# chairclr/PathTracing

Hardware: AMD Instinct MI355X
Metric: Mrays/s (higher is better)
Workload: dtype f32

## Files before the change

pathtracing_amd/csrc/kernels.hip:

```cpp
#include "ptrt_internal.h"
#include "pt_device.h"
#include <algorithm>
#include <cstdlib>


using namespace ptd;

namespace ptrt {

PT_DEV uint32_t lane_prefix(uint64_t m) { return __builtin_amdgcn_mbcnt_hi((uint32_t)(m >> 32), __builtin_amdgcn_mbcnt_lo((uint32_t)m, 0u)); }
PT_DEV uint32_t lane_id() { return lane_prefix(~0ull); }

typedef const float4 __attribute__((address_space(4))) *uniform_f4;
PT_DEV uniform_f4 as_uniform(const float4 *p) { return (uniform_f4)(uintptr_t)p; }
PT_DEV float4 uniform_load(uniform_f4 p, uint32_t i) { return make_float4(p[i].x, p[i].y, p[i].z, p[i].w); }
PT_DEV uint32_t spheres_test(const float4 *spheres, uint32_t n_spheres, uint32_t first_id, V3 o, V3 d, Hit &h)
{
    const uniform_f4 sp = as_uniform(spheres);
    for (uint32_t j = 0; j < n_spheres; j += 4u) {
        const float4 s0 = uniform_load(sp, j), s1 = uniform_load(sp, j + 1u), s2 = uniform_load(sp, j + 2u), s3 = uniform_load(sp, j + 3u);
        sphere_test(s0, first_id + j, o, d, h);
        if (j + 1u < n_spheres) sphere_test(s1, first_id + j + 1u, o, d, h);
        if (j + 2u < n_spheres) sphere_test(s2, first_id + j + 2u, o, d, h);
        if (j + 3u < n_spheres) sphere_test(s3, first_id + j + 3u, o, d, h);
// ... 300 lines not shown
    const bool in_range = j < ps.shard_cap && slot < ps.n_slots;
    const uint32_t first = first_sample(slot, fp);
    const bool valid = in_range && first < fp.spp && slot_pixel(slot, fp, x, y);
    if (in_range && !fp.accumulate) ps.acc[slot] = make_float4(0.f, 0.f, 0.f, 0.f);
    if (valid && full == 1u) {
        PathRegs r;
        path_init(sc, fp, slot, r);
        path_store(ps, slot, r);
    }
    if (full == 2u) wave_push(&ps.counters[cnt_ext_index(0, shard)], ps.q_ext[0] + (size_t)shard * ps.shard_cap, valid, slot);
    else if (j < ps.shard_cap) ps.q_ext[0][(size_t)shard * ps.shard_cap + j] = valid ? slot : kInvalidSlot;
    const uint32_t n_alive = (uint32_t)__syncthreads_count(valid);
    if (threadIdx.x == 0) {
        if (n_alive) atomicAdd(&ps.counters[cnt_alive_index(0, shard)], n_alive);
        if (bx == 0 && full != 2u) ps.counters[cnt_ext_index(0, shard)] = ps.shard_cap;
    }
}


template <int MODE>
PT_DEV bool shade_one(const DeviceScene &sc, const PathState &ps, const FrameParams &fp, uint32_t slot, PathRegs &r, float t, uint32_t ref,
                      uint32_t b, uint32_t &defer)
{
    V3 &o = r.o, &d = r.d, &T = r.T;
    uint32_t &key = r.key, &sample = r.sample;
    uint32_t depth = r.depth + 1u;
    float4 A = at(ps.acc, slot);
    bool touched = false, term = false, alive = false;
    auto add = [&](V3 L) {
        touched = true;
        A.x = fma_(T.x, L.x, A.x); A.y = fma_(T.y, L.y, A.y); A.z = fma_(T.z, L.z, A.z);
    };

    if (ref == PT_MISS) {
        add(v3(sc.sky[0], sc.sky[1], sc.sky[2]));
        term = true;
    } else {
        const V3 P = madd(t, d, o);
        V3 ng;
        uint32_t mat;
        if (ref < sc.n_tris) {
            const float4 ts = sc.tris[(size_t)ref * 4 + 3];
            ng = xyz(ts);
            mat = __float_as_uint(ts.w);
        } else {
            const uint32_t j = ref - sc.n_tris;
            const float4 s = sc.spheres[j];
            const uint2 mi = sc.sph_mat[j];
            const float ir = __uint_as_float(mi.y);
            ng = v3((P.x - s.x) * ir, (P.y - s.y) * ir, (P.z - s.z) * ir);
            mat = mi.x;
        }
        const bool front = dot(ng, d) < 0.0f;
        const V3 n = front ? ng : neg(ng);
        float4 m0 = sc.mats[(size_t)mat * 3], m1 = sc.mats[(size_t)mat * 3 + 1];
        const float4 m2 = sc.mats[(size_t)mat * 3 + 2];
        asm volatile("" : "+v"(m0.x), "+v"(m1.x));
        const V3 alb = v3(m0.y, m0.z, m0.w), emi = xyz(m1);
        const uint32_t kind = __float_as_uint(m0.x);
        if (MODE == SHADE_QUEUE && kind != (uint32_t)PT_LAMBERT) { defer = 1u + kind; return false; }
        if (emi.x != 0.0f || emi.y != 0.0f || emi.z != 0.0f) add(emi);
        if (depth >= fp.max_depth) term = true;
        else {
            const uint32_t bb = depth - 1u;
            const uint32_t bk = MODE == SHADE_QUEUE ? (uint32_t)B_LAMBERT : MODE == SHADE_BUCKETS ? b : 1u + kind;
            BsdfSample bs;
            if (bk == B_LAMBERT) bs = sample_lambert(alb, n, u01(key, 4u + 4u * bb), u01(key, 5u + 4u * bb));
            else if (bk == B_METAL) bs = sample_metal(alb, m1.w, d, n, u01(key, 4u + 4u * bb), u01(key, 5u + 4u * bb));
            else bs = sample_dielectric(alb, m2.x, d, n, front, u01(key, 6u + 4u * bb));
            const V3 wi = bs.wi, W = bs.W;
            const float side = bs.side;
            if (!bs.ok) term = true;
            else {
                T = v3(T.x * W.x, T.y * W.y, T.z * W.z);
                if (!(fmax_(T.x, fmax_(T.y, T.z)) > 0.0f)) term = true;
                else if (depth >= fp.rr_start) {
                    const float qrr = fmin_(fmax_(T.x, fmax_(T.y, T.z)), 0.95f);
                    if (!(u01(key, 7u + 4u * bb) < qrr)) term = true;
                    else { const float iq = 1.0f / qrr; T = v3(T.x * iq, T.y * iq, T.z * iq); }
                }
                if (!term) { o = madd(side * fp.ray_eps, n, P); d = wi; }
            }
        }
    }

    if (term) {
        touched = true;
        A.w += 1.0f;
        sample += fp.streams;
        if (sample < fp.spp) {
            uint32_t x = 0, y = 0;
            slot_pixel(slot, fp, x, y);
            key = path_key(fp.seed_hashed, y * fp.width + x, fp.sample_offset + sample);
            camera_ray_of(sc.cam, x, y, key, o, d);
            T = v3(1.f, 1.f, 1.f);
            depth = 0;
            alive = true;
        }
    } else alive = true;
    if (touched) at(ps.acc, slot) = A;
    r.depth = depth;
    return alive;
}

PT_DEV unsigned long long *traced_counter(const PathState &ps, uint32_t c, uint32_t shard)
{
    return reinterpret_cast<unsigned long long *>(ps.counters + cnt_traced_index(c, shard));
}
PT_DEV void fold_traced(const PathState &ps, uint32_t shard, uint32_t it, uint32_t n, uint32_t n_alive)
{
    *traced_counter(ps, (it + 2u) % 3u, shard) = 0ull;
    const unsigned long long traced = *traced_counter(ps, it % 3u, shard);
    *reinterpret_cast<unsigned long long *>(ps.counters + cnt_rays_index(shard)) += traced;
    if (ps.host_ring && it) ps.host_ring[((it - 1u) % ps.ring_slots) * kShards + shard] = make_uint4(n, n_alive, (uint32_t)traced, (uint32_t)(traced >> 32));
}

PT_DEV bool want_compact(const PathState &ps, uint32_t len, uint32_t n_alive, uint32_t prev_alive, bool sticky, bool forced)
{
    const uint32_t deaths = prev_alive > n_alive ? prev_alive - n_alive : 0u;
    const uint32_t predicted = n_alive > deaths ? n_alive - deaths : 0u;
    return forced || (sticky && len < ps.shard_cap) || (float)predicted < ps.compact_below * (float)len;
}

PT_DEV void queue_next(const PathState &ps, uint32_t shard, uint32_t cnext, uint32_t *q_next, uint32_t gid, uint32_t total, bool alive,
                       uint32_t slot, bool compact)
{
    if (compact) wave_push(&ps.counters[cnt_ext_index(cnext, shard)], q_next, alive, slot);
    else {
        if (gid < total) at(q_next, gid) = alive ? slot : kInvalidSlot;
        if (gid == 0) ps.counters[cnt_ext_index(cnext, shard)] = total;
    }
    const uint64_t m = __ballot(alive);
    if (m && lane_id() == 0u) atomicAdd(&ps.counters[cnt_alive_index(cnext, shard)], (uint32_t)__popcll(m));
}

#ifndef PT_EXT_WAVES
#define PT_EXT_WAVES(L, FUSE) (((L) == PT_BVH_WIDTH_4Q || (L) == PT_BVH_WIDTH_2) && (FUSE) != SHADE_INLINE ? 8 : 7)
#endif
struct StackCtx { int32_t *lds; uint32_t stride, tid, col; };
PT_DEV void push_slow(const StackCtx &k, uint32_t &sp, int32_t v)
{
    if (sp < kStackLds) k.lds[sp * k.stride + k.tid] = v;
    else {
        const PathState &ps = cold().ps;
        const uint32_t e = sp - kStackLds;
        if (e < ps.stack_ovf_entries) ps.stack_ovf[(size_t)e * ((size_t)kShards * ps.shard_cap) + k.col] = v;
        else { atomicOr(&ps.counters[kCntError], 1u); return; }
    }
    ++sp;
}
PT_DEV int32_t pop_slow(const StackCtx &k, uint32_t &sp)
{
    if (sp == 0) return PT_BVH_EMPTY;
    --sp;
    if (sp < kStackLds) return k.lds[sp * k.stride + k.tid];
    const PathState &ps = cold().ps;
    return ps.stack_ovf[(size_t)(sp - kStackLds) * ((size_t)kShards * ps.shard_cap) + k.col];
}
PT_DEV int32_t pop_lds(const StackCtx &k, uint32_t &sp)
{
    if (sp == 0) return PT_BVH_EMPTY;
    --sp;
    return k.lds[sp * k.stride + k.tid];
}
PT_DEV int32_t pop_after_leaf(const StackCtx &k, uint32_t &sp)
{
    const bool deep = __any((int)(sp > kStackLds)) != 0;
    return deep ? pop_slow(k, sp) : pop_lds(k, sp);
}

template <int L>
PT_DEV void node_visit_rows(const float4 *__restrict__ base, float4 r0, float4 r1, float4 r2, float4 r3, const StackCtx &k, const RaySetup &rs,
                            float t_best, int32_t &cur, uint32_t &sp);
template <int L>
PT_DEV void node_step(const float4 *__restrict__ nodes, const StackCtx &k, const RaySetup &rs, float t_best, int32_t &cur, uint32_t &sp)
{
    const float4 *base = nodes + (size_t)cur * node_rows<L>();
    node_visit_rows<L>(base, base[0], base[1], base[2], base[3], k, rs, t_best, cur, sp);
}
template <int L>
PT_DEV void node_visit_rows(const float4 *__restrict__ base, float4 r0, float4 r1, float4 r2, float4 r3, const StackCtx &k, const RaySetup &rs,
                            float t_best, int32_t &cur, uint32_t &sp)
{
    constexpr int N = fanout<L>();
    const bool deep = __any((int)(sp + (uint32_t)(N - 1) > kStackLds)) != 0;
    if constexpr (L == PT_BVH_WIDTH_8O) {
        uint32_t hits;
        int32_t ref[N];
        visit_node_oct8(base, r0, r1, r2, r3, rs, t_best, hits, ref);
        int32_t prev = PT_BVH_EMPTY;
        if (!deep) {
#pragma unroll
            for (int p = N - 1; p >= 0; --p) {
                const bool h = (hits >> p) & 1u;
                k.lds[sp * k.stride + k.tid] = prev;
                sp += (h && prev != PT_BVH_EMPTY) ? 1u : 0u;
                prev = h ? ref[p] : prev;
            }
            cur = prev != PT_BVH_EMPTY ? prev : pop_lds(k, sp);
        } else {
#pragma unroll
            for (int p = N - 1; p >= 0; --p)
                if ((hits >> p) & 1u) { if (prev != PT_BVH_EMPTY) push_slow(k, sp, prev); prev = ref[p]; }
            cur = prev != PT_BVH_EMPTY ? prev : pop_slow(k, sp);
        }
        return;
    }
    uint32_t key[N];
    int32_t ref[N];
    visit_node<L>(base, r0, r1, r2, r3, rs, t_best, key, ref);
    if (!deep) {
#pragma unroll
        for (int i = N - 1; i >= 1; --i) {
            k.lds[sp * k.stride + k.tid] = ref[i];
            sp += key[i] != 0xFFFFFFFFu ? 1u : 0u;
        }
        cur = key[0] != 0xFFFFFFFFu ? ref[0] : pop_lds(k, sp);
    } else {
#pragma unroll
        for (int i = N - 1; i >= 1; --i)
            if (key[i] != 0xFFFFFFFFu) push_slow(k, sp, ref[i]);
        cur = (key[0] != 0xFFFFFFFFu) ? ref[0] : pop_slow(k, sp);
    }
}

PT_DEV uint32_t leaf_step(const float4 *__restrict__ tris, const StackCtx &k, V3 o, V3 d, Hit &h, int32_t &cur, uint32_t &sp)
{
    const uint32_t enc = (uint32_t)~cur;
    uint32_t first = enc >> 3, more = enc & 7u, n = 0;
    for (;;) {
        const float4 *base = tris + (size_t)first * 4;
        const float4 r0 = base[0], r1 = base[1], r2 = base[2];
        tri_test(r0, r1, r2, first, o, d, h);
        ++n;
        if (more == 0u) break;
        ++first; --more;
    }
    cur = pop_after_leaf(k, sp);
    return n;
}

constexpr uint32_t kFinishVertices = 256;

struct ExtHead {
    uint32_t shard, bx, parity, cnext, n, n_alive;
    bool do_compact, idle;
};
template <int FUSE>
PT_DEV ExtHead extend_head(const ExtArgs &a, const PathState &ps, uint32_t per_block, uint32_t tid, bool predicted, bool carry_len)
{
    ExtHead e;
    const uint32_t it = a.it, ccur = it % 3u, czero = (it + 2u) % 3u;
    e.parity = it & 1u; e.cnext = (it + 1u) % 3u;
    uint32_t nbx;
    block_pos(a.ps, e.shard, e.bx, nbx);
    e.n = ps.counters[cnt_ext_index(ccur, e.shard)]; e.n_alive = ps.counters[cnt_alive_index(ccur, e.shard)];
    e.do_compact = FUSE != SHADE_NONE &&
                   (predicted ? want_compact(ps, e.n, e.n_alive, ps.counters[cnt_prev_alive_index(ccur, e.shard)], ps.repack_sticky != 0u, a.compact != 0u)
                              : want_compact(ps, e.n, e.n_alive, 0u, false, a.compact != 0u));
    if (e.bx * per_block + tid == 0u) {
        ps.counters[cnt_prev_alive_index(e.cnext, e.shard)] = e.n_alive;
        ps.counters[cnt_ext_index(czero, e.shard)] = 0u;
        ps.counters[cnt_alive_index(czero, e.shard)] = 0u;
        fold_traced(ps, e.shard, it, e.n, e.n_alive);
        if (FUSE == SHADE_NONE) *traced_counter(ps, e.cnext, e.shard) = e.n_alive;
        else if (carry_len && !e.do_compact) ps.counters[cnt_ext_index(e.cnext, e.shard)] = e.n;
        if (e.do_compact && e.n_alive) atomicAdd(&ps.counters[kCntCompactions], 1u);
    }
    e.idle = e.bx * per_block >= e.n || e.n_alive == 0u;
    return e;
}

PT_DEV void stash_park(uint32_t *stash, uint32_t stride, uint32_t tid, const PathRegs &r)
{
    stash[0 * stride + tid] = __float_as_uint(r.T.x); stash[1 * stride + tid] = __float_as_uint(r.T.y);
    stash[2 * stride + tid] = __float_as_uint(r.T.z); stash[3 * stride + tid] = r.key;
    stash[4 * stride + tid] = (r.sample << 8) | r.depth;
    asm volatile("" ::: "memory");
}
PT_DEV void stash_restore(const uint32_t *stash, uint32_t stride, uint32_t tid, PathRegs &r)
{
    r.T = v3(__uint_as_float(stash[0 * stride + tid]), __uint_as_float(stash[1 * stride + tid]), __uint_as_float(stash[2 * stride + tid]));
    r.key = stash[3 * stride + tid];
    const uint32_t sdv = stash[4 * stride + tid];
    r.sample = sdv >> 8; r.depth = sdv & 255u;
}

struct VisitCounts {
    unsigned long long nodes = 0, tris = 0, sph = 0;
    unsigned long long wave_iters = 0, wave_iters_late = 0, idle_leaf = 0, idle_done = 0;
};
PT_DEV void flush_visit_counters(const PathState &ps, const VisitCounts &v)
{
    auto add = [&](uint32_t i, unsigned long long x) { atomicAdd(reinterpret_cast<unsigned long long *>(ps.counters + i), x); };
    if (v.wave_iters) add(kCntWaveNodeIters, v.wave_iters);
    if (v.wave_iters_late) add(kCntWaveNodeIters + 2, v.wave_iters_late);
    if (v.idle_leaf) add(kCntIdleLeaf, v.idle_leaf);
    if (v.idle_done) add(kCntIdleDone, v.idle_done);
    add(kCntNodes, v.nodes);
    add(kCntTris, v.tris);
    add(kCntSph, v.sph);
}

template <int L, bool COUNT, int FUSE>
__global__ void __launch_bounds__(kExtBlock) __attribute__((amdgpu_waves_per_eu(PT_EXT_WAVES(L, FUSE), PT_EXT_WAVES(L, FUSE)))) k_extend(ExtArgs a)
{
    const float4 *__restrict__ nodes = a.sc.nodes, *__restrict__ tris = a.sc.tris, *__restrict__ spheres = a.sc.spheres;
    const uint32_t n_spheres = a.sc.n_spheres, n_tris = a.sc.n_tris, n_nodes = a.sc.n_nodes;
    const uint32_t it = a.it;
    __shared__ int32_t s_stack[kStackLds * kExtBlock];
    __shared__ uint32_t s_stash[(FUSE != SHADE_NONE ? 5 : 1) * kExtBlock];
    const uint32_t tid = threadIdx.x;
    ExtHead hd;
    uint32_t gid, qbase, slot = kInvalidSlot, n_bounces;
    {
        const PathState &ps = cold().ps;
        hd = extend_head<FUSE>(a, ps, kExtBlock, tid, true, false);
        gid = hd.bx * kExtBlock + tid;
        if (hd.idle) return;
        qbase = hd.shard * ps.shard_cap;
        if (gid < hd.n) slot = at(ps.q_ext[hd.parity], qbase + gid);
        const bool sparse = hd.do_compact && (float)hd.n_alive < ps.sparse_below * (float)hd.n;
        n_bounces = FUSE == SHADE_NONE ? 1u : (hd.n_alive <= ps.finish_below ? kFinishVertices : sparse ? 1u : a.bounces);
    }
    const uint32_t shard = hd.shard, parity = hd.parity, n = hd.n;
    const bool active = slot != kInvalidSlot;
    const StackCtx stk{ s_stack, kExtBlock, tid, qbase + gid };

    VisitCounts vc;
    __shared__ int32_t s_state[COUNT ? 64 : 1];
    PathRegs r;
    r.o = v3(0.f, 0.f, 0.f); r.d = v3(0.f, 0.f, 1.f); r.T = v3(0.f, 0.f, 0.f); r.key = r.sample = r.depth = 0u;
    if (active) {
        const PathState &ps = cold().ps;
        if (FUSE == SHADE_NONE) { r.o = xyz(at(ps.ray_o, slot)); r.d = xyz(at(ps.ray_d, slot)); }
        else if (it == 0u) {
            path_init(cold().sc, cold().fp, slot, r);
            if (!cold().fp.accumulate) at(ps.acc, slot) = make_float4(0.f, 0.f, 0.f, 0.f);
        }
        else path_load(ps, slot, r);
    }
    bool alive = active;
    uint32_t wave_rays = 0;
    for (uint32_t bounce = 0; bounce < n_bounces; ++bounce) {
    const uint64_t alive_mask = __ballot(alive);
    if (alive_mask == 0) break;
    wave_rays += (uint32_t)__popcll(alive_mask);
    if (COUNT && kExtBlock == 64u) { s_state[tid] = alive ? 0 : 1; __syncthreads(); }
    if (alive) {
        const V3 o = r.o, d = r.d;
        Hit h{ __builtin_inff(), PT_MISS, PT_MISS };
        if (FUSE != SHADE_NONE) stash_park(s_stash, kExtBlock, tid, r);

        { const uint32_t ns = spheres_test(spheres, n_spheres, n_tris, o, d, h); if (COUNT) vc.sph += ns; }

        const RaySetup rs = ray_setup(o, d);
        int32_t cur = n_nodes ? 0 : PT_BVH_EMPTY;
        uint32_t sp = 0, steps = 0;
        if (n_nodes) {
            ++steps;
            if (COUNT) { vc.nodes++; if (lane_id() == (uint32_t)(__ffsll((long long)__ballot(1)) - 1)) vc.wave_iters++; }
            const uniform_f4 root = as_uniform(nodes);
            node_visit_rows<L>(nodes, uniform_load(root, 0), uniform_load(root, 1), uniform_load(root, 2), uniform_load(root, 3), stk, rs, h.t, cur, sp);
            if (COUNT) s_state[tid & 63u] = cur;
        }

        bool late_cycle = false;
        for (;;) {
            while ((uint32_t)cur < (uint32_t)PT_BVH_EMPTY) {
                if (++steps > (1u << 22)) { atomicOr(&cold().ps.counters[kCntError], 2u); cur = PT_BVH_EMPTY; break; }
                if (COUNT) {
                    vc.nodes++;
                    if (lane_id() == (uint32_t)(__ffsll((long long)__ballot(1)) - 1)) {
                        vc.wave_iters++; if (late_cycle) vc.wave_iters_late++;
                        uint32_t n_leaf = 0, n_done = 0;
                        for (uint32_t l = 0; l < 64u; ++l) { const int32_t c2 = s_state[l]; n_leaf += c2 < 0 ? 1u : 0u; n_done += c2 == PT_BVH_EMPTY ? 1u : 0u; }
                        vc.idle_leaf += n_leaf; vc.idle_done += n_done;
                    }
                }
                node_step<L>(nodes, stk, rs, h.t, cur, sp);
                if (COUNT) s_state[tid & 63u] = cur;
            }
            if (cur == PT_BVH_EMPTY) break;
            if (COUNT) late_cycle = true;
            const uint32_t nt = leaf_step(tris, stk, o, d, h, cur, sp);
            if (COUNT) { vc.tris += nt; s_state[tid & 63u] = cur; }
        }

        if (FUSE == SHADE_NONE) at(cold().ps.hit, slot) = make_float2(h.t, __uint_as_float(h.ref));
        else {
            stash_restore(s_stash, kExtBlock, tid, r);
            uint32_t defer = 0u;
            const ExtArgs &c = cold();
            alive = shade_one<FUSE>(c.sc, c.ps, c.fp, slot, r, h.t, h.ref, B_LAMBERT, defer);
        }
    }
    }
    const PathState &ps = cold().ps;
    if (COUNT && active) flush_visit_counters(ps, vc);
    if (FUSE != SHADE_NONE) {
        if (alive) path_store(ps, slot, r);
        queue_next(ps, shard, hd.cnext, &at(ps.q_ext[parity ^ 1u], qbase), gid, n, alive, slot, hd.do_compact);
        if (wave_rays && lane_id() == 0u) atomicAdd(traced_counter(ps, hd.cnext, shard), (unsigned long long)wave_rays);
    }
}


#ifndef PT_REFILL_IDLE
#define PT_REFILL_IDLE 16
#endif
constexpr uint32_t kRefillIdle = PT_REFILL_IDLE;

#ifndef PT_PACKED_WAVES
#define PT_PACKED_WAVES(FUSE) ((FUSE) == SHADE_INLINE ? 6 : 7)
#endif
template <int L, bool COUNT, int FUSE>
__global__ void __launch_bounds__(64) __attribute__((amdgpu_waves_per_eu(PT_PACKED_WAVES(FUSE), PT_PACKED_WAVES(FUSE))))
k_extend_packed(ExtArgs a)
{
    const float4 *__restrict__ nodes = a.sc.nodes, *__restrict__ tris = a.sc.tris, *__restrict__ spheres = a.sc.spheres;
    const uint32_t n_spheres = a.sc.n_spheres, n_tris = a.sc.n_tris, n_nodes = a.sc.n_nodes;
    const uint32_t it = a.it, chunk = a.chunk, bounces = a.bounces;
    __shared__ int32_t s_stack[kStackLds * 64];
    __shared__ uint32_t s_stash[(FUSE != SHADE_NONE ? 5 : 1) * 64];
    const uint32_t lane = threadIdx.x;
    const ExtHead hd = extend_head<FUSE>(a, cold().ps, chunk, lane, false, true);
    if (hd.idle) return;
    const uint32_t shard = hd.shard, n_alive = hd.n_alive;
    const bool do_compact = hd.do_compact;
    uint32_t next = hd.bx * chunk;
    const uint32_t end = min(hd.n, next + chunk);
    const uint32_t qbase = hd.shard * cold().ps.shard_cap;
    const uint32_t *queue = cold().ps.q_ext[hd.parity] + (size_t)qbase;
    uint32_t *q_next = cold().ps.q_ext[hd.parity ^ 1u] + (size_t)qbase;
    const StackCtx stk{ s_stack, 64u, lane, qbase + hd.bx * 64u + lane };
    const uint32_t budget0 = FUSE == SHADE_NONE ? 1u : (n_alive <= cold().ps.finish_below ? kFinishVertices : bounces);

    bool has = false;
    uint32_t slot = 0, pos = 0, budget = 0, sp = 0, steps = 0;
    int32_t cur = PT_BVH_EMPTY;
    PathRegs r;
    r.o = v3(0.f, 0.f, 0.f); r.d = v3(0.f, 0.f, 1.f); r.T = v3(0.f, 0.f, 0.f); r.key = r.sample = r.depth = 0u;
    V3 &o = r.o, &d = r.d;
    RaySetup rs = ray_setup(o, d);
    Hit h{ __builtin_inff(), PT_MISS, PT_MISS };
    VisitCounts vc;
    uint32_t wave_rays = 0, wave_alive = 0;

    auto start_ray = [&]() {
        if (FUSE != SHADE_NONE) stash_park(s_stash, 64u, lane, r);
        h = Hit{ __builtin_inff(), PT_MISS, PT_MISS };
        { const uint32_t ns = spheres_test(spheres, n_spheres, n_tris, o, d, h); if (COUNT) vc.sph += ns; }
        rs = ray_setup(o, d);
        cur = n_nodes ? 0 : PT_BVH_EMPTY;
        sp = 0; steps = 0;
    };

    for (;;) {
        const bool fin = has && cur == PT_BVH_EMPTY;
        bool retired = false, retire_alive = false;
        if (fin) {
            if (FUSE == SHADE_NONE) {
                at(cold().ps.hit, slot) = make_float2(h.t, __uint_as_float(h.ref));
                has = false;
            } else {
                stash_restore(s_stash, 64u, lane, r);
                uint32_t defer = 0u;
                const bool alive = shade_one<FUSE>(cold().sc, cold().ps, cold().fp, slot, r, h.t, h.ref, B_LAMBERT, defer);
                --budget;
                if (alive && budget != 0u) start_ray();
                else {
                    if (alive) path_store(cold().ps, slot, r);
                    retired = true; retire_alive = alive; has = false;
                }
            }
        }
        if (FUSE != SHADE_NONE) {
            wave_rays += (uint32_t)__popcll(__ballot(fin && has));
            wave_alive += (uint32_t)__popcll(__ballot(retire_alive));
            if (do_compact) wave_push(&cold().ps.counters[cnt_ext_index(hd.cnext, shard)], q_next, retire_alive, slot);
            else if (retired) q_next[pos] = retire_alive ? slot : kInvalidSlot;
        }
        const uint64_t idle = __ballot(!has);
        const uint32_t avail = end - next;
        if (idle && avail) {
            const uint32_t prefix = lane_prefix(idle);
            const bool pull = !has && prefix < avail;
            if (pull) { pos = next + prefix; slot = queue[pos]; }
            if (pull && slot == kInvalidSlot) {
                if (FUSE != SHADE_NONE && !do_compact) q_next[pos] = kInvalidSlot;
            } else if (pull) {
                if (FUSE == SHADE_NONE) { o = xyz(at(cold().ps.ray_o, slot)); d = xyz(at(cold().ps.ray_d, slot)); }
                else if (it == 0u) {
                    path_init(cold().sc, cold().fp, slot, r);
                    if (!cold().fp.accumulate) at(cold().ps.acc, slot) = make_float4(0.f, 0.f, 0.f, 0.f);
                }
                else path_load(cold().ps, slot, r);
                budget = budget0;
                start_ray();
                has = true;
            }
            if (FUSE != SHADE_NONE) wave_rays += (uint32_t)__popcll(__ballot(pull && has));
            next += min((uint32_t)__popcll(idle), avail);
        }
        if (!__ballot(has)) {
            if (next < end) continue;
            break;
        }
        const uint32_t want = (next < end) ? kRefillIdle : 64u;
        for (;;) {
            if (cur != PT_BVH_EMPTY) {
                const bool inner = cur >= 0;
                const uint32_t enc = (uint32_t)~cur, first = enc >> 3, more = enc & 7u;
                const float4 *base = inner ? nodes + (size_t)cur * node_rows<L>() : tris + (size_t)first * 4;
                const float4 r0 = base[0], r1 = base[1], r2 = base[2], r3 = base[3];
                if (++steps > (1u << 22)) { atomicOr(&cold().ps.counters[kCntError], 2u); cur = PT_BVH_EMPTY; }
                else if (inner) {
                    node_visit_rows<L>(base, r0, r1, r2, r3, stk, rs, h.t, cur, sp);
                    if (COUNT) vc.nodes++;
                } else {
                    tri_test(r0, r1, r2, first, o, d, h);
                    if (COUNT) vc.tris++;
                    cur = more ? (int32_t)~(((first + 1u) << 3) | (more - 1u)) : pop_after_leaf(stk, sp);
                }
            }
            const uint32_t busy = (uint32_t)__popcll(__ballot(has && cur != PT_BVH_EMPTY));
            if (FUSE == SHADE_NONE) { if (busy == 0u || 64u - busy >= want) break; }
            else {
                const uint32_t waiting = (uint32_t)__popcll(__ballot(has && cur == PT_BVH_EMPTY));
                const uint32_t empty = (next < end) ? (uint32_t)__popcll(__ballot(!has)) : 0u;
                if (busy == 0u || waiting + empty >= kRefillIdle) break;
            }
        }
    }
    if (COUNT) flush_visit_counters(cold().ps, vc);
    if (FUSE != SHADE_NONE && lane == 0u) {
        if (wave_rays) atomicAdd(traced_counter(cold().ps, hd.cnext, shard), (unsigned long long)wave_rays);
        if (wave_alive) atomicAdd(&cold().ps.counters[cnt_alive_index(hd.cnext, shard)], wave_alive);
    }
}

#ifndef PT_POOL_WAVES
#define PT_POOL_WAVES(FUSE) ((FUSE) == SHADE_INLINE ? 6 : 7)
#endif
#ifndef PT_POOL_REFILL
#define PT_POOL_REFILL 16
#endif
#ifndef PT_POOL_LEAFWAIT
#define PT_POOL_LEAFWAIT 16
#endif
constexpr uint32_t kPoolRefill = PT_POOL_REFILL, kPoolLeafWait = PT_POOL_LEAFWAIT;

template <int L, bool COUNT, int FUSE>
__global__ void __launch_bounds__(64) __attribute__((amdgpu_waves_per_eu(PT_POOL_WAVES(FUSE), PT_POOL_WAVES(FUSE)))) k_extend_pool(ExtArgs a)
{
    static_assert(FUSE != SHADE_NONE, "the pool kernel always shades");
    constexpr uint32_t E = kPool, P = E / 64u;
    static_assert(E % 64u == 0 && E >= 64u && E <= 256u, "kPool: 64, 128, 192 or 256 (live list holds byte indices)");
    const float4 *__restrict__ nodes = a.sc.nodes, *__restrict__ tris = a.sc.tris, *__restrict__ spheres = a.sc.spheres;
    const uint32_t n_spheres = a.sc.n_spheres, n_tris = a.sc.n_tris, n_nodes = a.sc.n_nodes;
    __shared__ int32_t s_stack[kStackLds * 64];
    __shared__ float s_ht[E];
    __shared__ uint32_t s_href[E];
    __shared__ uint32_t s_slot[E];
    __shared__ uint8_t s_live[E];
    const uint32_t lane = threadIdx.x;
    ExtHead hd;
    uint32_t n_bounces;
    size_t qbase;
    {
        const PathState &ps = cold().ps;
        hd = extend_head<FUSE>(a, ps, E, lane, true, true);
        if (hd.idle) return;
        qbase = (size_t)hd.shard * ps.shard_cap;
        n_bounces = hd.n_alive <= ps.finish_below ? kFinishVertices : a.bounces;
    }
    const uint32_t shard = hd.shard, bx = hd.bx, parity = hd.parity, n = hd.n;
    const bool do_compact = hd.do_compact;
    const StackCtx stk{ s_stack, 64u, lane, (uint32_t)qbase + bx * 64u + lane };
    VisitCounts vc;

    auto spheres_of = [&](V3 o, V3 d, uint32_t e) {
        Hit h{ __builtin_inff(), PT_MISS, PT_MISS };
        spheres_test(spheres, n_spheres, n_tris, o, d, h);
        s_ht[e] = h.t; s_href[e] = h.ref;
    };
    auto live_append = [&](bool pred, uint32_t e, uint32_t &count) {
        const uint64_t m = __ballot(pred);
        if (pred) s_live[count + lane_prefix(m)] = (uint8_t)e;
        count += (uint32_t)__popcll(m);
    };

    uint32_t n_live = 0;
    {
        const PathState &ps = cold().ps;
#pragma unroll
        for (uint32_t hh = 0; hh < P; ++hh) {
            const uint32_t e = hh * 64u + lane, g = bx * E + e;
            const uint32_t slot = g < n ? ps.q_ext[parity][qbase + g] : kInvalidSlot;
            s_slot[e] = slot;
            const bool valid = slot != kInvalidSlot;
            if (valid) spheres_of(xyz(at(ps.ray_o, slot)), xyz(at(ps.ray_d, slot)), e);
            live_append(valid, e, n_live);
        }
    }
    __syncthreads();

    uint32_t wave_rays = 0;
    for (uint32_t bounce = 0; bounce < n_bounces && n_live; ++bounce) {
        wave_rays += n_live;
        uint32_t next = 0, e = 0, sp = 0, steps = 0;
        bool has = false;
        int32_t cur = PT_BVH_EMPTY;
        V3 o = v3(0.f, 0.f, 0.f), d = v3(0.f, 0.f, 1.f);
        RaySetup rs = ray_setup(o, d);
        Hit h{ __builtin_inff(), PT_MISS, PT_MISS };
        for (;;) {
            if (has && cur == PT_BVH_EMPTY) { s_ht[e] = h.t; s_href[e] = h.ref; has = false; }
            const uint64_t idle = __ballot(!has);
            const uint32_t avail = n_live - next;
            if (idle && avail) {
                const uint32_t prefix = lane_prefix(idle);
                if (!has && prefix < avail) {
                    const PathState &ps = cold().ps;
                    e = s_live[next + prefix];
                    const uint32_t slot = s_slot[e];
                    o = xyz(at(ps.ray_o, slot)); d = xyz(at(ps.ray_d, slot));
                    const uint32_t ref0 = s_href[e];
                    h = Hit{ s_ht[e], ref0, ref0 };
                    cur = n_nodes ? 0 : PT_BVH_EMPTY;
                    rs = ray_setup(o, d);
                    sp = 0; steps = 0; has = true;
                    if (COUNT) vc.sph += n_spheres;
                }
                next += min((uint32_t)__popcll(idle), avail);
            }
            if (!__ballot(has)) break;
            for (;;) {
                const bool is_n = has && (uint32_t)cur < (uint32_t)PT_BVH_EMPTY, is_l = has && cur < 0;
                const uint64_t m_n = __ballot(is_n), m_l = __ballot(is_l);
                if (!(m_n | m_l)) break;
                const uint32_t n_l = (uint32_t)__popcll(m_l), busy = (uint32_t)__popcll(m_n) + n_l;
                if (next < n_live && 64u - busy >= kPoolRefill) break;
                if (m_l && (!m_n || n_l >= kPoolLeafWait)) {
                    if (is_l) { const uint32_t nt = leaf_step(tris, stk, o, d, h, cur, sp); if (COUNT) vc.tris += nt; }
                } else if (is_n) {
                    if (++steps > (1u << 22)) { atomicOr(&cold().ps.counters[kCntError], 2u); cur = PT_BVH_EMPTY; }
                    else {
                        if (COUNT) { vc.nodes++; if (lane == (uint32_t)(__ffsll((long long)m_n) - 1)) vc.wave_iters++; }
                        node_step<L>(nodes, stk, rs, h.t, cur, sp);
                    }
                }
            }
        }
        __syncthreads();

        const bool last = bounce + 1u == n_bounces;
        uint32_t n_next = 0;
        const ExtArgs &c = cold();
#pragma unroll
        for (uint32_t hh = 0; hh < P; ++hh) {
            const uint32_t e2 = hh * 64u + lane;
            const uint32_t slot = s_slot[e2];
            bool alive = false;
            if (slot != kInvalidSlot) {
                PathRegs r;
                path_load(c.ps, slot, r);
                uint32_t defer = 0u;
                alive = shade_one<FUSE>(c.sc, c.ps, c.fp, slot, r, s_ht[e2], s_href[e2], B_LAMBERT, defer);
                if (alive) {
                    path_store(c.ps, slot, r);
                    if (!last) spheres_of(r.o, r.d, e2);
                } else s_slot[e2] = kInvalidSlot;
            }
            live_append(alive, e2, n_next);
        }
        n_live = n_next;
        __syncthreads();
    }

    const PathState &ps = cold().ps;
    uint32_t *q_next = ps.q_ext[parity ^ 1u] + qbase;
    uint32_t n_left = 0;
#pragma unroll
    for (uint32_t hh = 0; hh < P; ++hh) {
        const uint32_t e2 = hh * 64u + lane, g = bx * E + e2;
        const uint32_t slot = s_slot[e2];
        const bool alive = slot != kInvalidSlot;
        if (do_compact) wave_push(&ps.counters[cnt_ext_index(hd.cnext, shard)], q_next, alive, slot);
        else if (g < n) q_next[g] = slot;
        n_left += (uint32_t)__popcll(__ballot(alive));
    }
    if (COUNT) flush_visit_counters(ps, vc);
    if (lane == 0u) {
        if (wave_rays) atomicAdd(traced_counter(ps, hd.cnext, shard), (unsigned long long)wave_rays);
        if (n_left) atomicAdd(&ps.counters[cnt_alive_index(hd.cnext, shard)], n_left);
    }
}

enum TraceMode { TRACE_CLOSEST = 0, TRACE_COUNT = 1, TRACE_OCCLUSION = 2 };
struct TraceArgs : ExtArgs {
    const float4 *rays;
    float4 *hits;
    uint32_t n;
};
// ... 243 lines not shown
```

Before: 16850.

## Add fast path that retires leading sky-miss camera samples without full traversal

On the first iteration of the fused extend kernel, each camera ray is tested cheaply against the spheres and the BVH root node. While at least a threshold number of lanes in the wave have rays that miss everything, those lanes add the sky colour to the accumulator and generate their next sample in place. The aim is to skip full traversal and shading round-trips for primary rays that obviously hit nothing. In exchange it adds extra root tests on every first iteration, a divergent loop, and LDS atomics, and rays retired this way are counted into the traced-ray metric.

```diff
diff --git a/pathtracing_amd/csrc/kernels.hip b/pathtracing_amd/csrc/kernels.hip
--- a/pathtracing_amd/csrc/kernels.hip
+++ b/pathtracing_amd/csrc/kernels.hip
@@ -626,6 +626,64 @@
     add(kCntSph, v.sph);
 }
 
+#ifndef PT_MISS_STREAK_LANES
+#define PT_MISS_STREAK_LANES 32
+#endif
+constexpr uint32_t kMissStreakLanes = PT_MISS_STREAK_LANES;
+
+template <int L>
+PT_DEV bool ray_misses(V3 o, V3 d)
+{
+    Hit h{ __builtin_inff(), PT_MISS, PT_MISS };
+    const DeviceScene &sc = cold().sc;
+    spheres_test(sc.spheres, sc.n_spheres, sc.n_tris, o, d, h);
+    if (h.ref != PT_MISS) return false;
+    if (sc.n_nodes == 0u) return true;
+    const RaySetup rs = ray_setup(o, d);
+    const uniform_f4 root = as_uniform(sc.nodes);
+    const float4 r0 = uniform_load(root, 0), r1 = uniform_load(root, 1), r2 = uniform_load(root, 2), r3 = uniform_load(root, 3);
+    constexpr int N = fanout<L>();
+    int32_t ref[N];
+    if constexpr (L == PT_BVH_WIDTH_8O) {
+        uint32_t hits;
+        visit_node_oct8(sc.nodes, r0, r1, r2, r3, rs, h.t, hits, ref);
+        return hits == 0u;
+    } else {
+        uint32_t key[N];
+        visit_node_keys<L>(sc.nodes, r0, r1, r2, r3, rs, h.t, key, ref);
+        bool any = false;
+#pragma unroll
+        for (int c = 0; c < N; ++c) any |= key[c] != 0xFFFFFFFFu;
+        return !any;
+    }
+}
+
+template <int L>
+PT_DEV bool leading_misses(uint32_t slot, PathRegs &r, bool alive, uint32_t *rays)
+{
+    bool s = alive && ray_misses<L>(r.o, r.d);
+    if ((uint32_t)__popcll(__ballot(s)) < kMissStreakLanes) return alive;
+    float4 A = make_float4(0.f, 0.f, 0.f, 0.f);
+    if (s && cold().fp.accumulate) A = at(cold().ps.acc, slot);
+    uint32_t n = 0, x = 0, y = 0;
+    if (s) slot_pixel(slot, cold().fp, x, y);
+    while ((uint32_t)__popcll(__ballot(s)) >= kMissStreakLanes) {
+        if (!s) continue;
+        const ExtArgs &c = cold();
+        A.x = fma_(1.0f, c.sc.sky[0], A.x); A.y = fma_(1.0f, c.sc.sky[1], A.y); A.z = fma_(1.0f, c.sc.sky[2], A.z);
+        A.w += 1.0f;
+        ++n;
+        r.sample += c.fp.streams;
+        if (r.sample < c.fp.spp) {
+            r.key = path_key(c.fp.seed_hashed, y * c.fp.width + x, c.fp.sample_offset + r.sample);
+            camera_ray_of(c.sc.cam, x, y, r.key, r.o, r.d);
+            s = ray_misses<L>(r.o, r.d);
+        } else { alive = false; s = false; }
+    }
+    if (n) { at(cold().ps.acc, slot) = A; atomicAdd(rays, n); }
+    return alive;
+}
+
 template <int L, bool COUNT, int FUSE>
 __global__ void __launch_bounds__(kExtBlock) __attribute__((amdgpu_waves_per_eu(PT_EXT_WAVES(L, FUSE), PT_EXT_WAVES(L, FUSE)))) k_extend(ExtArgs a)
 {
@@ -664,7 +722,13 @@
         }
         else path_load(ps, slot, r);
     }
+    __shared__ uint32_t s_streak[kExtBlock / 64u];
     bool alive = active;
+    if constexpr (!COUNT && FUSE != SHADE_NONE)
+        if (it == 0u) {
+            if (lane_id() == 0u) s_streak[tid >> 6] = 0u;
+            alive = leading_misses<L>(slot, r, active, &s_streak[tid >> 6]);
+        }
     uint32_t wave_rays = 0;
     for (uint32_t bounce = 0; bounce < n_bounces; ++bounce) {
     const uint64_t alive_mask = __ballot(alive);
@@ -725,6 +789,7 @@
     if (FUSE != SHADE_NONE) {
         if (alive) path_store(ps, slot, r);
         queue_next(ps, shard, hd.cnext, &at(ps.q_ext[parity ^ 1u], qbase), gid, n, alive, slot, hd.do_compact);
+        if (!COUNT && it == 0u) wave_rays += s_streak[tid >> 6];
         if (wave_rays && lane_id() == 0u) atomicAdd(traced_counter(ps, hd.cnext, shard), (unsigned long long)wave_rays);
     }
 }
```

Measured after the change: 16890 (median of 6 runs). About the same (+0.3%).
